# bpp/bpp

Hardware: AMD Instinct MI355X
Metric: MCMC iterations/sec (A00) + site-lnL updates/sec, 10k loci, 1/2/4/8 GPU (higher is better)
Workload: dtype f64; 1 GPU; C2: A00, 10000 loci x 1000 sites, 4 taxa, JC69, 1 rate cat; 10000 loci on rank 0, 5.2 patterns/locus; parallelism=1 GPU, moves=program

## Files before the change

### bpp_amd/csrc/sweep2.hpp

```cpp
#pragma once

namespace smp2 {

using smp::Tree; using smp::Species; using smp::ByteArr; using smp::MAXPOP; using smp::MAXN;
using smp::rndu; using smp::reflect; using smp::msc_term; using smp::nth_bit; using smp::Op; using smp::make_op;

template <int NT> struct Cfg
{
  static constexpr int G     = NT <= 4 ? 8 : NT <= 8 ? 16 : 32;
  static constexpr int LPW   = 64/G;
  static constexpr int NN    = 2*NT;
  static constexpr int W     = NN/4;
  static constexpr int NBUF  = 2*(NT - 1);
  static constexpr int NPM   = 2*(2*NT - 2);
#ifndef SMP2_WAVES
#define SMP2_WAVES 8
#endif
  static constexpr int WAVES = NT <= 4 ? SMP2_WAVES : 4;
  static constexpr int BS    = 64*WAVES;
  static constexpr int PARK  = 28 + 4*W;
  static_assert(G == NN, "lane i of a group is node i");
};

struct Loc
// ... 32 lines not shown
  const Sched * sched; uint32_t sched_on;
  uint32_t xshards;
};

constexpr int XV = 15;
constexpr uint32_t XS_MIN = 8, XS_MAX = 64, XLINE = 16;
constexpr size_t XBUF_WORDS = (size_t)2*XS_MAX*XLINE;
constexpr int XSLEEP_FIRST = 16;
struct XLayout { uint32_t set_words, shard, word; };
__host__ __device__ inline XLayout xlayout(uint32_t S, uint32_t b, uint32_t lane, uint32_t load)
{
  XLayout L;
  L.set_words = S*XLINE;
  L.shard = (b & (S - 1u))*XLINE;
  L.word = ((lane >> 4) + 4u*load)*XLINE + (lane & 15u);
  return L;
}
template <int NL> __device__ __forceinline__ unsigned long long xpoll_sum(const unsigned long long * p, uint32_t step)
{
  unsigned long long v[NL];
#pragma unroll
  for (int j = 0; j < NL; ++j) v[j] = __hip_atomic_load(p + (size_t)j*step, __ATOMIC_RELAXED, __HIP_MEMORY_SCOPE_AGENT);
  unsigned long long s = v[0];
#pragma unroll
  for (int j = 1; j < NL; ++j) s += v[j];
  return s;
}

template <int NT> struct Slot
{
  double time[Cfg<NT>::NN];
  double ab[Cfg<NT>::NPM][2];
  double contrib[Cfg<NT>::G], contrib_new[Cfg<NT>::G];
  double rate, rw, f[4];
};
template <int NT> struct WaveLDS
{
  double clv[Cfg<NT>::NBUF][64][4];
  double term[64];
  uint2  pat[64];
  Slot<NT> slot[Cfg<NT>::LPW];
};
struct PopFit { double k, T, a, b, c; };
struct Redraw { double tn, l2t, T, a, b, c; };
struct WgBase
{
  double tau[3*MAXPOP];
  double xtot[32];
  Species sp;
  struct { unsigned long long grng; uint32_t accm, rd_mask, acc_step, run_ok; double lnacc_step, lnacc_theta; double tn[16], l2t[16], lnacc[16]; } dec;
  PopFit pf[16];
  Redraw rd[16];
  struct { int32_t q, mix; double tq_old, tq_lo, tq_hi, tq_new, minf, maxf, lminf, lmaxf, mix_c, mix_lnc; } stepp;
};
template <int NT> struct WgLDS : WgBase
{
  double lograt[(2*NT)*(2*NT)];
  unsigned long long accfx[32];
  uint32_t anc[16];
  uint32_t abort_, bad_, xbad_, coarse_;
  unsigned long long xprev[2][64];
  long long prof[24];
  long long wsweep[16];
  uint32_t roles[8];
  uint32_t xcoarse_, late_;
  uint32_t simd[8];
  uint32_t handoff[8][SCHED_SEGS];
  unsigned long long b1abs; long long hwait[8], b1last;
};

template <int G> __device__ __forceinline__ uint32_t gballot(bool p, uint32_t gbase)
{
  return (uint32_t)(__ballot(p) >> gbase) & (G >= 32 ? 0xffffffffu : ((1u << (G & 31)) - 1u));
}
__device__ __forceinline__ void wsync()
{
  __builtin_amdgcn_fence(__ATOMIC_ACQ_REL, "wavefront");
  __builtin_amdgcn_wave_barrier();
}

template <int NT> struct GTree
{
  ByteArr<Cfg<NT>::W> left, right, parent, pop;
  uint32_t cf, pf;
  int32_t root, tips;
  __device__ __forceinline__ int cidx(int i) const { return i + (((cf >> i) & 1u) ? tips - 1 : 0); }
  __device__ __forceinline__ int pidx(int i) const { return i + (((pf >> i) & 1u) ? 2*tips - 2 : 0); }
};

__device__ __forceinline__ uint32_t splat(int v) { return (uint32_t)(v & 0xff)*0x01010101u; }
__device__ __forceinline__ uint32_t byte_eq(uint32_t w, uint32_t s)
{
  const uint32_t x = w ^ s;
  const uint32_t z = ~(((x & 0x7f7f7f7fu) + 0x7f7f7f7fu) | x | 0x7f7f7f7fu);
  return (z - (z >> 7)) | z;
}
template <int NT> __device__ __forceinline__ void swap_ids(GTree<NT> & t, double * time, int a, int b)
{
  constexpr int W = Cfg<NT>::W;
  const uint32_t sa = splat(a), sb = splat(b), x = sa ^ sb;
#pragma unroll
  for (int k = 0; k < W; ++k)
  {
    t.left.w[k]   ^= x & (byte_eq(t.left.w[k], sa)   | byte_eq(t.left.w[k], sb));
    t.right.w[k]  ^= x & (byte_eq(t.right.w[k], sa)  | byte_eq(t.right.w[k], sb));
    t.parent.w[k] ^= x & (byte_eq(t.parent.w[k], sa) | byte_eq(t.parent.w[k], sb));
  }
  const int la = t.left[a], ra = t.right[a], pa = t.parent[a], qa = t.pop[a];
  const int lb = t.left[b], rb = t.right[b], pb = t.parent[b], qb = t.pop[b];
  t.left.set(a, lb); t.right.set(a, rb); t.parent.set(a, pb); t.pop.set(a, qb);
  t.left.set(b, la); t.right.set(b, ra); t.parent.set(b, pa); t.pop.set(b, qa);
  const double ta = time[a], tb = time[b];
  time[a] = tb; time[b] = ta;
  t.root = t.root == a ? b : t.root == b ? a : t.root;
}
template <int NT> __device__ __forceinline__ uint32_t path_mask(const GTree<NT> & t, int v)
{
  uint32_t m = 0;
#pragma unroll
  for (int d = 0; d < NT; ++d) { if (v >= 0) { m |= 1u << v; v = t.parent[v]; } }
  return m;
}

// ... 390 lines not shown
  const uint32_t lane = threadIdx.x & 63u, pl16 = lane & 15u, role = lane >> 4;
  const int npop = wg.sp.npop, pm = (int)pl16;
  const double qnan = prog_qnan();
  const bool run_ok = wg.dec.run_ok != 0u;
  const PopFit f = wg.pf[pl16];
  const bool have = lane < 32u && pm < npop && ((theta_mask >> pm) & 1u) && run_ok;
  const double Ts = f.T*mix_c;
  double fa = qnan, fb = qnan, tn = qnan, l2t = 0;
  if (have) theta_conditional<TK>(wg, f.k, role == 0u ? Ts : Ts/mix_c, &fa, &fb);
  const double fao = __shfl(fa, 16 + pm, 64), fbo = __shfl(fb, 16 + pm, 64);
  const uint32_t rd_mask = (uint32_t)__ballot(lane < 16u && have && fa == fa && fao == fao) & 0xffffu;
  double xl;
  const double s_fa = __shfl(fa, pm, 64), s_fb = __shfl(fb, pm, 64);
  const double g = draw_gammas<TK>(z, lane, 0xfedcba9876543210ull, npop, rd_mask, fa, role == 1u ? s_fb : role == 2u ? s_fa : fbo, xl);
  const double lb = __shfl(xl, 16 + pm, 64), la = __shfl(xl, 32 + pm, 64), lbo = __shfl(xl, 48 + pm, 64), lao = log(fao);
  const double c1 = fa*lb - lgamma_with_log(fa, la), co = fao*lbo - lgamma_with_log(fao, lao);
  if (lane < 16u && ((rd_mask >> pl16) & 1u)) tn = 1.0/(g/fb);
  const double x = redraw_ratio<TK>(wg, lane, f.k, tn, fa, fb, c1, Ts, fao, fbo, co, f.T, l2t);
  double lnacc_theta = 0;
  for (int p = 0; p < npop; ++p)
    if ((theta_mask >> p) & 1u)
    {
      const double xp = __shfl(x, p, 64);
      lnacc_theta += run_ok && ((rd_mask >> p) & 1u) ? xp : qnan;
    }
  if (lane < 16u) { Redraw & r = wg.rd[lane]; r.tn = tn; r.l2t = l2t; r.T = Ts; r.a = fa; r.b = fb; r.c = c1; }
  if (lane == 0) { wg.dec.rd_mask = rd_mask; wg.dec.lnacc_theta = lnacc_theta; }
  __builtin_amdgcn_fence(__ATOMIC_ACQ_REL, "wavefront");
  __builtin_amdgcn_wave_barrier();
  return z;
}

template <int NT, bool BPP, bool PROG = false, bool HO = false>
__global__ void __launch_bounds__(Cfg<NT>::BS) iter_kernel(const Args A)
{
  static_assert(!HO || PROG, "sets change waves in the program-moves kernel only");
  using C = Cfg<NT>;
  constexpr int G = C::G, LPW = C::LPW, NN = C::NN, W = C::W, NBUF = C::NBUF, NPM = C::NPM, WAVES = C::WAVES;
  extern __shared__ __attribute__((aligned(16))) unsigned char smem[];
  WgLDS<NT> & wg = *reinterpret_cast<WgLDS<NT> *>(smem);
  WaveLDS<NT> * wl_all = reinterpret_cast<WaveLDS<NT> *>(smem + ((sizeof(WgLDS<NT>) + 15) & ~(size_t)15));
  const uint32_t tid = threadIdx.x, wv = tid >> 6, lane = tid & 63u, b = blockIdx.x;
  const int li = (int)(lane & (uint32_t)(G - 1)); const uint32_t gbase = lane - (uint32_t)li, slot = lane/(uint32_t)G;
  const uint32_t lw = PROG ? wv - 1u : wv;
  WaveLDS<NT> * wl = wl_all + (PROG ? (wv && !(HO && wv > A.lwaves) ? wv - 1u : 0u) : wv);
  Slot<NT> * S = &wl->slot[slot];
  const uint32_t gw = lw < A.lwaves ? b*A.lwaves + lw : 0xffffffffu;
  {
    const uint32_t * src = reinterpret_cast<const uint32_t *>(A.sp);
    uint32_t * dst = reinterpret_cast<uint32_t *>(&wg.sp);
    for (uint32_t i = tid; i < sizeof(Species)/4; i += C::BS) dst[i] = src[i];
    if (tid < 24u) wg.prof[tid] = 0;
    if (tid < 16u) wg.wsweep[tid] = 0;
    if constexpr (HO)
    {
      if (tid < 8u) { wg.hwait[tid] = 0; wg.roles[tid] = 0xff0u; }
      if (tid < 8u*SCHED_SEGS) (&wg.handoff[0][0])[tid] = 0u;
      if (tid == 0) { wg.b1last = 0; wg.b1abs = 0ull; }
      if (lane == 0) wg.simd[wv & 7u] = (uint32_t)__builtin_amdgcn_s_getreg((1 << 11) | (4 << 6) | 4);
    }
  }
  __syncthreads();
  const Species & SP = wg.sp;
  const int npop = SP.npop, nsp = SP.S;

  for (uint32_t i = tid; i < (uint32_t)(3*MAXPOP); i += C::BS) wg.tau[i] = A.taus[i];
  for (uint32_t i = tid; i < (uint32_t)((2*NT)*(2*NT)); i += C::BS) wg.lograt[i] = A.lograt[(i/(2*NT))*MAXN + i % (2*NT)];
  if (tid < 16u) wg.anc[tid] = tid < (uint32_t)MAXPOP ? (uint32_t)SP.anc[tid] : 0u;
  if (tid == 0) { wg.abort_ = __hip_atomic_load(A.err, __ATOMIC_RELAXED, __HIP_MEMORY_SCOPE_AGENT) != 0 ? 2u : 0u; wg.late_ = 0; wg.bad_ = 0; wg.xbad_ = 0; wg.coarse_ = 0; wg.xcoarse_ = 0; }
  if (tid < 32u) wg.accfx[tid] = 0ull;
  if (tid < 2u*64u) (&wg.xprev[0][0])[tid] = 0ull;
  PopLane pl;
  {
    pl.parent = li < npop ? (int)SP.parent[li < MAXPOP ? li : 0] : -1;
    pl.anc = li < npop ? (uint32_t)SP.anc[li < MAXPOP ? li : 0] : 0u;
    uint32_t below = 0;
    for (int q2 = 0; q2 < npop; ++q2) if (q2 != li && (((uint32_t)SP.anc[q2] >> li) & 1u)) below |= 1u << q2;
    pl.below = li < npop ? below : 0u;
  }
  __syncthreads();
  if (wg.abort_ == 2u)
  {
    if (b == 0 && tid == 0) (void)atomicAdd(A.err + 1, (int)A.niter);
    return;
  }
  auto load_pop = [&]()
  {
    const int i = li < MAXPOP ? li : 0;
    pl.tau = wg.tau[i]; pl.theta = wg.tau[MAXPOP + i]; pl.l2t = wg.tau[2*MAXPOP + i];
    pl.ptau = pl.parent >= 0 ? wg.tau[pl.parent] : -1.0;
  };
  load_pop();
  Stream<BPP> grng{*A.grng};

  const bool prof_on = (A.dbg & 16u) && b == 0 && tid == 0;
  long long pf_t = prof_on ? clock64() : 0;
#define SMP2_TICK(i_) do { if (prof_on) { const long long t1_ = clock64(); wg.prof[i_] += t1_ - pf_t; pf_t = t1_; } } while (0)
  long long pf_s = 0;
#define SMP2_SUB0() do { if (prof_on) pf_s = clock64(); } while (0)
#define SMP2_SUB(i_) do { if (prof_on) wg.prof[i_] += clock64() - pf_s; } while (0)

  constexpr double FX = 1099511627776.0;
  constexpr double FXC = 1024.0;
  auto fx_add = [&](int v, double x, bool coarse)
  {
    if (fabs(x) < 256.0)
// ... 168 lines not shown
      uint32_t pj_tau = 0, pj_tau_acc = 0, pj_mix = 0, pj_mix_acc = 0;
      const bool declog = (A.dbg & 256u) && b == 0;
      int q = -1; bool mix = false;
      double tq_old = 0, tq_new = 0, mix_c = 1, mix_lnc = 0, lnprior = 0;
      auto make_step = [&](int stepq)
      {
        mix = stepq == npop; q = mix ? -1 : stepq;
        const double wprop = g.window();
        double tq_lo = 0, tq_hi = 0, minf = 1, maxf = 1, lminf = 0, lmaxf = 0;
        tq_old = 0; tq_new = 0; mix_c = 1; mix_lnc = 0; lnprior = 0;
        if (!mix)
        {
          const int pq = SP.parent[q], cl = SP.left[q], cr = SP.right[q];
          tq_old = wg.tau[q]; tq_lo = fmax(wg.tau[cl], wg.tau[cr]); tq_hi = pq >= 0 ? wg.tau[pq] : 999.0;
          tq_new = reflect(tq_old + SP.ft_tau*wprop, tq_lo, tq_hi);
          minf = (tq_new - tq_lo)/(tq_old - tq_lo); maxf = (tq_new - tq_hi)/(tq_old - tq_hi);
          const double lg = log(lane == 0 ? minf : lane == 1u ? maxf : tq_new/tq_old);
          lminf = __shfl(lg, 0, 64); lmaxf = __shfl(lg, 1, 64);
          if (pq < 0 && SP.tau_alpha > 0) lnprior = (SP.tau_alpha - 1 - (nsp - 1) + 1)*__shfl(lg, 2, 64) - SP.tau_beta*(tq_new - tq_old);
        }
        else { mix_lnc = SP.ft_mix*wprop; mix_c = exp(mix_lnc); }
        if (lane == 0)
        {
          wg.stepp.q = q; wg.stepp.mix = mix ? 1 : 0; wg.stepp.tq_old = tq_old; wg.stepp.tq_lo = tq_lo; wg.stepp.tq_hi = tq_hi; wg.stepp.tq_new = tq_new;
          wg.stepp.minf = minf; wg.stepp.maxf = maxf; wg.stepp.lminf = lminf; wg.stepp.lmaxf = lmaxf; wg.stepp.mix_c = mix_c; wg.stepp.mix_lnc = mix_lnc;
        }
      };
      uint32_t slidem = 0; double tslide = 0;
      auto theta_choices = [&]()
      {
        slidem = 0; tslide = 0;
        for (int p = 0; p < npop; ++p)
          if ((tm >> p) & 1u)
          {
            if (!(g.u() < SP.theta_slide_prob)) continue;
            slidem |= 1u << p;
            const double tn = reflect(wg.tau[MAXPOP + p] + SP.ft_theta*g.window(), 0.0, 999.0);
            if (p == (int)lane) tslide = tn;
          }
      };
      bool aborted = false;
      if (A.do_allloci && A.niter) { make_step(nsp); theta_choices(); }
      __syncthreads();
      for (uint32_t it = 0; it < A.niter && A.do_allloci && !aborted; ++it)
      {
        for (int stepq = nsp; stepq <= npop && !aborted; ++stepq)
        {
          const bool first = stepq == nsp;
          const int base = first ? nth : 0;
          if (mix) { SMP2_SUB0(); g.r = prog_mix_redraw((uint32_t)g.r, tm, mix_c); SMP2_SUB(15); }
          SMP2_TICK(0);
          __syncthreads();
          SMP2_TICK(1);
          if constexpr (HO) if (wg.abort_) { if (b == 0 && lane == 0) (void)atomicAdd(A.err + 1, (int)A.niter); aborted = true; __syncthreads(); __syncthreads(); break; }
          double dummy = 0;
          exchange_begin(base + (mix ? 2 : 5));
          SMP2_TICK(2);
          const bool okx = exchange_end(0, dummy);
          SMP2_TICK(3);
          if (!okx) { aborted = true; __syncthreads(); __syncthreads(); break; }
          if ((A.dbg & 64u) && A.world == 1)
          {
            xdummy = true; xrow = 16;
            exchange_begin(base + (mix ? 2 : 5));
            const bool okd = exchange_end(0, dummy);
            xdummy = false; xrow = 8;
            if (!okd) { aborted = true; __syncthreads(); __syncthreads(); break; }
            if (prof_on) pf_t = clock64();
          }
          bool accept = false; double lnacc = 0; uint32_t rd_mask = 0;
          if (first)
          {
            g.r = prog_theta_decide((uint32_t)g.r, tm, slidem, tslide, 1, q, base);
            const uint32_t accm = wg.dec.accm;
            cnt_prop += (uint32_t)__popc(tm); cnt_acc += (uint32_t)__popc(accm);
            cnt_gprop += (uint32_t)__popc(tm & ~slidem); cnt_gacc += (uint32_t)__popc(accm & tm & ~slidem);
            if (declog && lane < (uint32_t)npop && ((tm >> lane) & 1u))
            {
              const uint32_t k = ndec + (uint32_t)__popc(tm & ((1u << lane) - 1u));
              if (k < 1000u) { double * r = A.declog + 4*k; r[0] = (((slidem >> lane) & 1u) ? 100 : 200) + (int)lane; r[1] = wg.dec.lnacc[lane]; r[2] = -1.0; r[3] = (accm >> lane) & 1u ? 1 : 0; }
            }
            ndec += (uint32_t)__popc(tm);
            SMP2_TICK(4);
          }
          if (!mix)
          {
            g.r = prog_tau_decide((uint32_t)g.r, tm, q, base, lnprior, first);
            accept = wg.dec.acc_step != 0u; rd_mask = wg.dec.rd_mask; lnacc = wg.dec.lnacc_step;
          }
          else
          {
            lnacc = (wg.xtot[0] + wg.xtot[1]*(FX/FXC)) + (double)(nsp - 1)*mix_lnc;
            if (SP.tau_alpha > 0)
            {
              const double troot = wg.tau[npop - 1];
              lnacc += (SP.tau_alpha - 1)*mix_lnc - SP.tau_beta*(troot*mix_c - troot) - (double)(nsp - 2)*mix_lnc;
            }
            lnacc += wg.dec.lnacc_theta; rd_mask = wg.dec.rd_mask;
            accept = g.accept(lnacc);
            if (lane == 0) wg.dec.acc_step = accept ? 1u : 0u;
          }
          if (accept && wg.xcoarse_ && b == 0 && lane == 0) (void)atomicAdd(A.err + 2, 1);
          ++cnt_prop; cnt_acc += accept ? 1u : 0u;
          if (mix) { ++pj_mix; pj_mix_acc += accept ? 1u : 0u; } else { ++pj_tau; pj_tau_acc += accept ? 1u : 0u; }
          if (declog && lane == 0 && ndec < 1000u) { double * r = A.declog + 4*ndec; r[0] = mix ? 300 : 200 + q; r[1] = lnacc; r[2] = -1.0; r[3] = accept ? 1 : 0; }
          ++ndec;
          if (accept)
          {
            if (!mix) { if (lane == 0) wg.tau[q] = tq_new; }
            else if (lane < (uint32_t)npop) wg.tau[lane] *= mix_c;
            if (lane < 16u)
            {
              const Redraw r = wg.rd[lane];
              if ((rd_mask >> lane) & 1u) { wg.tau[MAXPOP + lane] = r.tn; wg.tau[2*MAXPOP + lane] = r.l2t; }
              const bool moved = mix ? lane < (uint32_t)npop && ((tm >> lane) & 1u)
                                     : ((tm >> lane) & 1u) && ((int)lane == q || (int)lane == SP.left[q] || (int)lane == SP.right[q]);
              if (moved) { PopFit & f = wg.pf[lane]; f.T = r.T; f.a = r.a; f.b = r.b; f.c = r.c; }
            }
          }
          wsync();
          if (mix) SMP2_TICK(6); else SMP2_TICK(5);
          SMP2_TICK(7);
          __syncthreads();
          if (stepq < npop) make_step(stepq + 1);
          else if (it + 1 < A.niter) { make_step(nsp); theta_choices(); }
          __syncthreads();
        }
      }
      if (!aborted)
      {
        if (lane == 0) wg.late_ = __hip_atomic_load(A.err, __ATOMIC_ACQUIRE, __HIP_MEMORY_SCOPE_AGENT) != 0 ? 1u : 0u;
        __syncthreads();
        if (wg.late_) { aborted = true; if (b == 0 && lane == 0) (void)atomicAdd(A.err + 1, (int)A.niter); }
      }
      if (b == 0)
      {
        if (lane == 0 && !aborted)
        {
          *A.grng = g.r;
          A.counters[0] += cnt_prop; A.counters[1] += cnt_acc; A.counters[2] += cnt_gprop; A.counters[3] += cnt_gacc;
          A.pj[4] += pj_tau; A.pj[5] += pj_tau_acc; A.pj[6] += pj_mix; A.pj[7] += pj_mix_acc;
          A.pj[8] += (cnt_prop - pj_tau - pj_mix) - cnt_gprop; A.pj[9] += (cnt_acc - pj_tau_acc - pj_mix_acc) - cnt_gacc;
        }
        if (!aborted && lane < (uint32_t)(3*MAXPOP)) A.taus[lane] = wg.tau[lane];
        if (prof_on) for (int i = 0; i < 24; ++i) A.prof[(i < 16 ? 0 : (int)A.nwg) + i] = (double)wg.prof[i];
        if (prof_on) for (int i = 0; i < 16; ++i) A.prof[(int)A.nwg + 24 + i] = (double)wg.wsweep[i];
        if (HO && prof_on) { for (int i = 0; i < 8; ++i) { A.prof[(int)A.nwg + 40 + i] = (double)wg.hwait[i]; A.prof[(int)A.nwg + 49 + i] = (double)wg.roles[i]; } A.prof[(int)A.nwg + 48] = (double)wg.b1last; }
      }
      return;
    }
  }

  const uint32_t t0 = gw < A.nwaves ? A.wave_off[gw] : 0u, nt = gw < A.nwaves ? A.wave_off[gw + 1] - t0 : 0u;
  bool act = slot < nt;
  uint32_t task = t0 + (act ? slot : 0u);
  GTree<NT> T;
  Stream<BPP> rng{0};
  double lnl_cur = 0, logpr_cur = 0;
  uint32_t np = 0, pb = 0, nprop_done = 0, nacc = 0, w_nupd = 0, w_nbr = 0, a_nupd = 0, a_nbr = 0, a_neval = 0;
  int gl_i = 0;
  for (int k = 0; k < W; ++k) { T.left.w[k] = T.right.w[k] = T.parent.w[k] = T.pop.w[k] = 0xffffffffu; }
  T.cf = T.pf = 0; T.root = 0; T.tips = 2;
  if (act && nt)
  {
    const Loc & L = A.loc[task];
    const uint32_t flag_now = __hip_atomic_load(A.mix_flag, __ATOMIC_RELAXED, __HIP_MEMORY_SCOPE_AGENT);
    const bool restore_mix = A.epoch != 0u && flag_now == A.epoch;
    const Tree * trp = A.trees + task;
    if (restore_mix) trp = A.snap + task;
    const Tree & tr = *trp;
    const Tree & cur = A.trees[task];
    np = L.np;
    double * g_pmat = L.pmat;
    if (li == 0) { S->rate = L.rate; S->rw = L.rw; S->f[0] = L.f0; S->f[1] = L.f1; S->f[2] = L.f2; S->f[3] = L.f3; }
    gl_i = L.gl[li & 15];
    for (int k = 0; k < W; ++k)
    {
      T.left.w[k] = reinterpret_cast<const uint32_t *>(tr.left)[k]; T.right.w[k] = reinterpret_cast<const uint32_t *>(tr.right)[k];
      T.parent.w[k] = reinterpret_cast<const uint32_t *>(tr.parent)[k]; T.pop.w[k] = reinterpret_cast<const uint32_t *>(tr.pop)[k];
// ... 2 lines not shown
    const int n = 2*T.tips - 1;
    T.cf = gballot<G>(li >= T.tips && li < n && tr.clv[li] != li, gbase);
    T.pf = gballot<G>(li < n && tr.pmat[li] != li, gbase);
    S->time[li] = li < n ? tr.time[li] : 0.0;
    for (uint32_t i = (uint32_t)li; i < (uint32_t)(4*(2*T.tips - 2)); i += G) (&S->ab[0][0])[i] = g_pmat[i];
  }
  {
    uint32_t acc = 0;
#pragma unroll
    for (int s2 = 0; s2 < LPW; ++s2)
    {
      const uint32_t n2 = (uint32_t)__builtin_amdgcn_readlane((int)np, s2*G);
      if ((uint32_t)s2 == slot) pb = acc;
      acc += n2;
    }
  }
  if (act)
  {
    const Loc & L = A.loc[task];
    const double * g_clv = L.clv;
    for (uint32_t q = (uint32_t)li; q < np; q += G) wl->pat[pb + q] = A.pat[L.pat_off + q];
    const uint32_t nbuf = 2u*(uint32_t)(T.tips - 1);
    for (uint32_t i = (uint32_t)li; i < nbuf*np; i += G)
    {
      const uint32_t c = i/np, q = i - c*np;
      const double2 * src = reinterpret_cast<const double2 *>(g_clv + ((size_t)c*np + q)*4);
      const double2 u = src[0], w = src[1];
      double * d = wl->clv[c][pb + q];
      d[0] = u.x; d[1] = u.y; d[2] = w.x; d[3] = w.y;
    }
  }
  int tips = T.tips, n = 2*tips - 1;
  bool inner_i = li >= tips && li < n;

  uint32_t mync = 0; double t2h_cur = 0, t2h_new = 0;
  uint32_t mynodes = 0, mync_new = 0; int mynin_new = 0;
  Op opw[NT - 1]; int nops = 0;
  for (int k = 0; k < NT - 1; ++k) opw[k] = 0;

  auto density_counts = [&]()
  {
    const int pop_i = T.pop[li];
    int below = 0;
#pragma unroll
    for (int q = 0; q < G - 1; ++q)
    {
      const uint32_t m = gballot<G>(inner_i && pop_i == q, gbase);
      if (li == q) mynodes = m;
      below += ((pl.below >> q) & 1u) ? __popc(m) : 0;
    }
    mync_new = (uint32_t)__popc(mynodes);
    mynin_new = gl_i - below;
  };
  auto density_term = [&](const double * tk)
  {
    uint32_t nodes = mynodes;
    const int ncoal = (int)mync_new, nin = mynin_new;
    int steps = ncoal + (pl.ptau >= 0 ? 1 : 0);
    if (nin == steps) --steps;
    double T2h = 0, prev = pl.tau;
    int nn = nin;
#pragma unroll
    for (int k = 0; k < NT; ++k)
      if (k < steps)
      {
        double tkk = pl.ptau;
        if (k < ncoal)
        {
          int best = -1; double tb = 0;
#pragma unroll
          for (int j = 0; j < NT - 1; ++j)
            if (((nodes >> (tips + j)) & 1u) && (best < 0 || tk[j] < tb)) { best = tips + j; tb = tk[j]; }
          tkk = tb; nodes &= ~(1u << best);
        }
        T2h += nn*(nn - 1)*(tkk - prev);
        prev = tkk; --nn;
      }
    double c = 0;
    if (ncoal) c += ncoal*pl.l2t;
    if (T2h) c -= T2h/(pl.theta*1.0);
    S->contrib_new[li] = c; t2h_new = T2h;
  };
  auto evaluate = [&](const Prop & pr, bool with_lnl, double & lp_new) -> double
  {
    double tk[NT - 1];
#pragma unroll
    for (int j = 0; j < NT - 1; ++j) tk[j] = S->time[(tips + j) & (NN - 1)];
    const double myage = S->time[li];
    density_counts();
    if ((pr.chain >> li) & 1u) density_term(tk);
    T.pf ^= pr.brm; T.cf ^= pr.ndm;
    if ((pr.brm >> li) & 1u)
    {
      const int par = T.parent[li];
      const double len = (S->time[par & (NN - 1)] - myage)*1.0;
      double a_, b_;
      jc69_ab(len, S->rate, a_, b_);
      const int pi = T.pidx(li);
      S->ab[pi][0] = a_; S->ab[pi][1] = b_;
    }
    nops = __popc(pr.ndm);
    {
      int rank = 0;
#pragma unroll
      for (int j = 0; j < NT - 1; ++j)
        rank += (((pr.ndm >> (tips + j)) & 1u) && (tk[j] < myage || (tk[j] == myage && tips + j < li))) ? 1 : 0;
      const bool mine = (pr.ndm >> li) & 1u;
#pragma unroll
      for (int k = 0; k < NT - 1; ++k)
        if (k < nops)
        {
          const int x = __ffs(gballot<G>(mine && rank == k, gbase)) - 1;
          const int l = T.left[x], r = T.right[x];
          opw[k] = make_op(T.cidx(x), T.cidx(l), T.pidx(l), T.cidx(r), T.pidx(r));
        }
    }
    wsync();
    double lnl = 0;
    if (with_lnl)
    {
      for (uint32_t base = 0; base < np; base += G)
      {
        const uint32_t q = base + (uint32_t)li; const bool pact = q < np;
        const uint32_t ps = pb + (pact ? q : 0u);
        const uint2 pi = wl->pat[ps];
        double last[4] = {0, 0, 0, 0}; uint32_t last_c = 0xffffffffu;
#pragma unroll
        for (int k = 0; k < NT - 1; ++k)
          if (k < nops)
          {
            const Op o = opw[k];
            const uint32_t opar = (uint32_t)o & 255u, lc = (uint32_t)(o >> 8) & 255u, lp = (uint32_t)(o >> 16) & 255u,
                           rc = (uint32_t)(o >> 24) & 255u, rp = (uint32_t)(o >> 32) & 255u;
            double lv[4], rv[4], x[4], y[4];
            if (lc < (uint32_t)tips) expand_code((pi.y >> (4*lc)) & 15u, lv);
            else if (lc == last_c) { lv[0] = last[0]; lv[1] = last[1]; lv[2] = last[2]; lv[3] = last[3]; }
            else { const double * c = wl->clv[lc - tips][ps]; lv[0] = c[0]; lv[1] = c[1]; lv[2] = c[2]; lv[3] = c[3]; }
            if (rc < (uint32_t)tips) expand_code((pi.y >> (4*rc)) & 15u, rv);
            else if (rc == last_c) { rv[0] = last[0]; rv[1] = last[1]; rv[2] = last[2]; rv[3] = last[3]; }
            else { const double * c = wl->clv[rc - tips][ps]; rv[0] = c[0]; rv[1] = c[1]; rv[2] = c[2]; rv[3] = c[3]; }
            matvec4_ab(S->ab[lp][0], S->ab[lp][1], lv, x);
            matvec4_ab(S->ab[rp][0], S->ab[rp][1], rv, y);
            last[0] = x[0]*y[0]; last[1] = x[1]*y[1]; last[2] = x[2]*y[2]; last[3] = x[3]*y[3]; last_c = opar;
            if (pact) { double * out = wl->clv[opar - tips][ps]; out[0] = last[0]; out[1] = last[1]; out[2] = last[2]; out[3] = last[3]; }
          }
        const double tr_ = dot4_pair(S->f[0], S->f[1], S->f[2], S->f[3], last);
        if (pact) wl->term[ps] = log(0 + tr_*S->rw)*pi.x;
      }
      wsync();
      for (uint32_t base = 0; base < np; base += 8)
      {
        double v[8];
#pragma unroll
        for (int j = 0; j < 8; ++j) v[j] = base + (uint32_t)j < np ? wl->term[pb + base + (uint32_t)j] : 0.0;
#pragma unroll
        for (int j = 0; j < 8; ++j) lnl += v[j];
      }
      lnl = A.bfbeta == 1.0 ? lnl : A.bfbeta == 0.0 ? 0.0 : A.bfbeta*lnl;
    }
    else wsync();
    double lp = 0;
    {
      double v[G];
#pragma unroll
      for (int p = 0; p < G; ++p) v[p] = p < npop ? (((pr.chain >> p) & 1u) ? S->contrib_new[p] : S->contrib[p]) : 0.0;
#pragma unroll
      for (int p = 0; p < G; ++p) lp += v[p];
    }
    lp_new = lp;
    return lnl;
  };
  auto commit_density = [&](uint32_t chain)
  {
    if ((chain >> li) & 1u) { S->contrib[li] = S->contrib_new[li]; t2h_cur = t2h_new; }
    mync = mync_new;
  };

  const uint32_t allpop = (1u << npop) - 1u;
  if (act)
  {
    wsync();
    double tk[NT - 1];
#pragma unroll
    for (int j = 0; j < NT - 1; ++j) tk[j] = S->time[(tips + j) & (NN - 1)];
    density_counts();
    if (li < npop) density_term(tk);
    commit_density(allpop);
    wsync();
    if (A.refresh_logpr)
    {
      double lp = 0;
      for (int p = 0; p < npop; ++p) lp += S->contrib[p];
      logpr_cur = lp;
    }
  }

  const double qnan = __longlong_as_double(0x7ff8000000000000ll);
  uint32_t cnt_prop = 0, cnt_acc = 0;
  uint32_t cnt_gprop = 0, cnt_gacc = 0;
  uint32_t pj_tau = 0, pj_tau_acc = 0, pj_mix = 0, pj_mix_acc = 0, pj_gage = 0, pj_gage_acc = 0;
  uint32_t step = 0;

  if constexpr (HO)
  {
    uint32_t role = 0xffu; bool handover = false;
    if (A.sched_on && lw < A.lwaves && A.lwaves <= 7u)
    {
      const uint32_t L = A.lwaves;
      uint32_t nalone = 0; bool valid = true;
      for (uint32_t x = 0; x < L; ++x)
      {
        uint32_t cnt = 0;
        for (uint32_t y = 0; y < L; ++y) cnt += (y != x && wg.simd[y + 1u] == wg.simd[x + 1u]) ? 1u : 0u;
        valid = valid && cnt <= 1u;
        nalone += cnt == 0u ? 1u : 0u;
      }
      uint32_t ia = 0, ip = 0;
      for (uint32_t x = 0; x < L; ++x)
      {
        int partner = -1;
        for (uint32_t y = 0; y < L; ++y) if (y != x && wg.simd[y + 1u] == wg.simd[x + 1u]) partner = (int)y;
        if (partner < 0) { if (x == lw) role = ia; ++ia; }
        else if ((uint32_t)partner > x)
        {
          if (x == lw) role = nalone + 2u*ip;
          if ((uint32_t)partner == lw) role = nalone + 2u*ip + 1u;
          ++ip;
        }
      }
      handover = valid && ip == (uint32_t)A.sched->npairs && nalone + 2u*ip == (uint32_t)A.sched->nroles && role < 8u;
    }
    if (lane == 0) wg.roles[wv & 7u] = wg.simd[wv & 7u] | (role << 4) | (handover ? 0x1000u : 0u);
    wsync();
  }
  auto park = [&]()
  {
    if constexpr (HO) {
    const uint32_t myset = (uint32_t)(wl - wl_all);
    uint32_t * r = reinterpret_cast<uint32_t *>(wl_all + A.lwaves) + (size_t)myset*(C::PARK*64) + lane;
// ... 55 lines not shown
      act = false;
      if (lane == 0) wg.roles[wv & 7u] &= ~0x1000u;
    }
    wsync();
    }
  };
  auto segment_begin = [&](uint32_t seg, uint32_t it, uint32_t nprop, bool prof) -> uint32_t
  {
    if constexpr (HO)
    {
      const uint32_t role = (wg.roles[wv & 7u] >> 4) & 7u;
      const uint32_t nseg = A.sched->nseg, src = A.sched->src[role][seg & 3u], nrun = A.sched->n[role][seg & 3u];
      if (seg && src != role) hand_over(role, src, seg, it, prof);
      return (wg.roles[wv & 7u] & 0x1000u) && seg + 1u < nseg && step + nrun < nprop ? step + nrun : nprop;
    }
    return nprop;
  };
  const bool declog = (A.dbg & 256u) && b == 0;
  uint32_t ndec = 0;
  const bool wgprof = (A.dbg & 32u) && tid == 0;
  long long wg_sweep = 0;
  bool aborted = false;

  if constexpr (PROG) __syncthreads();
  for (uint32_t it = 0; it < A.niter && !aborted; ++it)
  {
    const uint32_t nprop = HO && lw >= A.lwaves ? 0u : A.nsteps_gage + A.nsteps_gspr;
    const long long wg_t0 = wgprof ? clock64() : 0;
    const bool wvprof = (A.dbg & 16u) && b == 0 && lane == 0;
    const long long wv_t0 = wvprof ? clock64() : 0;
    step = 0;
    uint32_t seg = 0;
    do
    {
    uint32_t seg_end = nprop;
    if constexpr (HO) { if (wg.roles[wv & 7u] & 0x1000u) seg_end = segment_begin(seg, it, nprop, wvprof); ++seg; }
    for (; step < seg_end; ++step)
    {
      const GTree<NT> U = T;
      double tsave = 0, lnl = 0, lp_new = 0;
      Prop pr{0, 0, 0, 0.0};
      bool ok = false;
      if (act)
      {
        tsave = S->time[li];
        ok = step < A.nsteps_gage
          ? propose_gage<NT, BPP>(T, rng, S->time, (int)step, pl, wg.anc, wg.tau, SP.ft_gage, li, gbase, pr)
          : propose_gspr<NT, BPP>(T, rng, S->time, (int)(step - A.nsteps_gage), pl, gl_i, wg.anc, wg.tau, wg.lograt, SP.ft_gspr, li, gbase, pr);
      }
      SMP2_TICK(0);
      if (ok)
      {
        wsync();
        lnl = evaluate(pr, true, lp_new);
        SMP2_TICK(1);
      }
      if (ok)
      {
        w_nupd += (uint32_t)nops; w_nbr += (uint32_t)__popc(pr.brm);
        const double lnacc = (lp_new - logpr_cur) + (lnl - lnl_cur) + pr.hast;
        ++nprop_done;
        const bool gage_step = step < A.nsteps_gage;
        pj_gage += gage_step ? 1u : 0u;
        if (rng.accept(lnacc)) { lnl_cur = lnl; logpr_cur = lp_new; ++nacc; pj_gage_acc += gage_step ? 1u : 0u; commit_density(pr.chain); }
        else { T = U; S->time[li] = tsave; }
        wsync();
        SMP2_TICK(2);
      }
      else if (act) { T = U; S->time[li] = tsave; wsync(); }
    }
    } while (HO && step < nprop);
    (void)seg;
    if (wgprof) wg_sweep += clock64() - wg_t0;
    if (wvprof)
    {
      const long long t1 = clock64();
      wg.wsweep[wv] += t1 - wv_t0;
      if constexpr (HO) (void)__hip_atomic_fetch_max(&wg.b1abs, (unsigned long long)t1, __ATOMIC_RELAXED, __HIP_MEMORY_SCOPE_WORKGROUP);
    }
    if (!A.do_allloci) continue;

    constexpr bool program = PROG;
    bool mix = false; int q = -1;
    double wprop = 0, uacc = -1.0;
    double tq_old = 0, tq_lo = 0, tq_hi = 0, minf = 1, maxf = 1, lminf = 0, lmaxf = 0, tq_new = 0, mix_c = 1, mix_lnc = 0;
    double lnacc_theta = 0;
    double rd_tn = qnan, rd_l2t = 0, rd_T = 0, rd_a = qnan, rd_b = qnan, rd_c = qnan;
    uint32_t rd_mask = 0;
    uint32_t cf0 = 0, pf0 = 0;
    double tsave = 0, lnl_new = 0, lp_new = 0, lnprior = 0, dl_tot = 0, lnacc = 0;
    bool evaluated = false, accept = false;
    auto step_begin = [&](int stepq)
    {
      rd_mask = 0; lnprior = 0; accept = false; lnacc_theta = 0;
      if constexpr (PROG)
      {
        (void)stepq;
        mix = wg.stepp.mix != 0; q = wg.stepp.q;
        tq_old = wg.stepp.tq_old; tq_lo = wg.stepp.tq_lo; tq_hi = wg.stepp.tq_hi; tq_new = wg.stepp.tq_new;
        minf = wg.stepp.minf; maxf = wg.stepp.maxf; lminf = wg.stepp.lminf; lmaxf = wg.stepp.lmaxf; mix_c = wg.stepp.mix_c; mix_lnc = wg.stepp.mix_lnc;
      }
      else
      {
        mix = stepq == npop;
        q = mix ? -1 : stepq;
        wprop = mix && !BPP ? grng.u() - 0.5 : grng.window(); uacc = BPP ? -1.0 : grng.u();
        tq_old = 0; tq_lo = 0; tq_hi = 0; minf = 1; maxf = 1; lminf = 0; lmaxf = 0; tq_new = 0; mix_c = 1; mix_lnc = 0;
        if (!mix)
        {
          const int pq = SP.parent[q], cl = SP.left[q], cr = SP.right[q];
          tq_old = wg.tau[q]; tq_lo = fmax(wg.tau[cl], wg.tau[cr]); tq_hi = pq >= 0 ? wg.tau[pq] : 999.0;
          tq_new = reflect(tq_old + SP.ft_tau*wprop, tq_lo, tq_hi);
          minf = (tq_new - tq_lo)/(tq_old - tq_lo); maxf = (tq_new - tq_hi)/(tq_old - tq_hi);
          lminf = log(minf); lmaxf = log(maxf);
        }
        else { mix_lnc = SP.ft_mix*wprop; mix_c = exp(mix_lnc); }
      }
      if (!mix)
      {
        if (li == q) pl.tau = tq_new;
        if (pl.parent == q) pl.ptau = tq_new;
      }
      else
      {
        pl.tau *= mix_c;
        if (pl.parent >= 0) pl.ptau *= mix_c;
      }
    };
    auto step_locus = [&](int base)
    {
      cf0 = T.cf; pf0 = T.pf;
      tsave = act ? S->time[li] : 0.0;
      lnl_new = lnl_cur; lp_new = logpr_cur;
      evaluated = false;
      if (act)
      {
        Prop pr{allpop, 0, 0, 0.0};
        double hast = 0, hast2 = 0;
        if (!mix)
        {
          const int cl = SP.left[q], cr = SP.right[q];
          const int pk = T.pop[li];
          const double tk_ = tsave;
          const bool moved = inner_i && (pk == q || pk == cl || pk == cr) && !(tk_ < tq_lo || tk_ > tq_hi);
          const bool up = moved && tk_ >= tq_old;
          if (moved) S->time[li] = up ? tq_hi + maxf*(tk_ - tq_hi) : tq_lo + minf*(tk_ - tq_lo);
          const uint32_t mm = gballot<G>(moved, gbase);
          const int above = __popc(gballot<G>(up, gbase)), below = __popc(mm) - above;
          const int par = T.parent[li];
          pr.brm = gballot<G>(li < n && par >= 0 && (((mm >> li) & 1u) || ((mm >> (par & 31)) & 1u)), gbase);
          uint32_t m = mm;
          const int l = T.left[li], r = T.right[li];
#pragma unroll
          for (int d = 0; d < NT - 2; ++d) m |= gballot<G>(inner_i && (((m >> (l & 31)) & 1u) || ((m >> (r & 31)) & 1u)), gbase);
          pr.ndm = m;
          hast = below*lminf; hast2 = above*lmaxf;
        }
        else
        {
          if (inner_i) S->time[li] = tsave*mix_c;
          pr.ndm = gballot<G>(inner_i, gbase);
          pr.brm = gballot<G>(li < n && (int)T.parent[li] >= 0, gbase);
          hast = (double)(tips - 1)*mix_lnc;
        }
        wsync();
        evaluated = pr.ndm != 0;
        const double lnl = evaluate(pr, evaluated, lp_new);
        if (evaluated) { lnl_new = lnl; a_nupd += (uint32_t)nops; a_nbr += (uint32_t)__popc(pr.brm); ++a_neval; }
        const double dpr = program ? 0.0 : lp_new - logpr_cur;
        const double h = mix ? dpr + hast : (dpr + hast) + hast2;
        const double dl = evaluated ? (lnl_new - lnl_cur) + h : h;
        if (li == 0) fx_add(base, dl, true);
        if (program && !mix && li < npop && ((A.theta_mask >> li) & 1u))
        {
          const int slot = li == q ? 2 : li == SP.left[q] ? 3 : li == SP.right[q] ? 4 : -1;
          if (slot >= 0) fx_add(base + slot, t2h_new, false);
        }
      }
    };
    auto step_decide = [&](int base)
    {
      dl_tot = wg.xtot[base] + wg.xtot[base + 1]*(FX/FXC);
      lnacc = dl_tot;
      if (!mix) lnacc += lnprior;
      else
      {
        lnacc += (double)(nsp - 1)*mix_lnc;
        if (SP.tau_alpha > 0)
        {
          const double troot = wg.tau[npop - 1];
          lnacc += (SP.tau_alpha - 1)*mix_lnc - SP.tau_beta*(troot*mix_c - troot) - (double)(nsp - 2)*mix_lnc;
        }
      }
      accept = BPP ? grng.accept(lnacc) : (lnacc >= 0 || uacc < exp(lnacc));
    };
    auto step_apply = [&](bool refresh)
    {
      if constexpr (!PROG)
      {
        if (accept && wg.xcoarse_ && b == 0 && tid == 0) (void)atomicAdd(A.err + 2, 1);
        ++cnt_prop; cnt_acc += accept ? 1u : 0u;
        if (mix) { ++pj_mix; pj_mix_acc += accept ? 1u : 0u; } else { ++pj_tau; pj_tau_acc += accept ? 1u : 0u; }
        if (declog && tid == 0 && ndec < 1000u) { double * r = A.declog + 4*ndec; r[0] = mix ? 300 : 200 + q; r[1] = lnacc; r[2] = uacc; r[3] = accept ? 1 : 0; }
        ++ndec;
        __syncthreads();
        if (accept)
        {
          if (!mix) { if (tid == 0) wg.tau[q] = tq_new; }
          else if (tid < (uint32_t)npop) wg.tau[tid] *= mix_c;
        }
      }
      if (accept) { if (act) { lnl_cur = lnl_new; logpr_cur = lp_new; commit_density(allpop); } }
      else if (act) { T.cf = cf0; T.pf = pf0; S->time[li] = tsave; }
      if constexpr (!PROG) __syncthreads();
      load_pop();
      wsync();
      if (PROG && (refresh || accept) && act)
      {
        if (li < npop) S->contrib[li] = msc_term((int)mync, t2h_cur, pl.theta, pl.l2t);
        wsync();
        double lp = 0;
        for (int p = 0; p < npop; ++p) lp += S->contrib[p];
        logpr_cur = lp;
        wsync();
      }
    };
    if constexpr (PROG)
    {
      const bool on = li < npop && ((A.theta_mask >> li) & 1u);
      const int kidx = __popc(A.theta_mask & ((1u << li) - 1u)), nth = 2*__popc(A.theta_mask);
      for (int stepq = nsp; stepq <= npop && !aborted; ++stepq)
      {
        const bool first = stepq == nsp;
        step_begin(stepq);
        if (first && act && on) { fx_add(2*kidx, (double)mync, false); fx_add(2*kidx + 1, t2h_cur, false); }
        step_locus(first ? nth : 0);
        __syncthreads();
        if constexpr (HO) if (first && wvprof && lw == 0u) wg.b1last += (long long)wg.b1abs - wv_t0;
        __syncthreads();
        const bool ab = wg.abort_ != 0u;
        accept = wg.dec.acc_step != 0u;
        if (!ab) step_apply(first);
        __syncthreads();
        if (ab) { aborted = true; break; }
      }
    }
    else
    {
    if (SP.theta_alpha > 0 && A.theta_mask)
    {
      const bool on = li < npop && ((A.theta_mask >> li) & 1u);
      const double told = pl.theta, l2t_old = pl.l2t;
      double tnew = told, uacc = -1.0, my_lnacc = 0;
      bool accept = false, gibbs_me = false;
      {
        double win = 0;
        for (int p = 0; p < npop; ++p)
          if ((A.theta_mask >> p) & 1u)
          {
            const double w_ = grng.window(), a_ = BPP ? -1.0 : grng.u();
            if (p == li) { win = w_; uacc = a_; }
          }
        tnew = reflect(told + SP.ft_theta*win, 0.0, 999.0);
        const double l2t_new = log(2.0/(1.0*tnew));
        if (act && on) fx_add(li, msc_term((int)mync, t2h_cur, tnew, l2t_new) - msc_term((int)mync, t2h_cur, told, l2t_old), false);
        SMP2_TICK(3);
        double th_tot = 0;
        if (!exchange(npop, li, th_tot)) { aborted = true; break; }
        SMP2_TICK(6);
        if (BPP)
        {
          if (on) { wl->term[li] = tnew; wl->term[16 + li] = told; }
          wsync();
          for (int p = 0; p < npop; ++p)
            if ((A.theta_mask >> p) & 1u)
            {
              const double tn = wl->term[p], to = wl->term[16 + p];
              const double lnacc = wg.xtot[p] + ((SP.theta_alpha - 1)*log(tn/to) - SP.theta_beta*(tn - to));
              const bool acc = tn > 0 && grng.accept(lnacc);
              if (p == li) { accept = acc; my_lnacc = lnacc; }
            }
          wsync();
        }
        else if (on)
        {
          my_lnacc = th_tot + ((SP.theta_alpha - 1)*log(tnew/told) - SP.theta_beta*(tnew - told));
          accept = tnew > 0 && (my_lnacc >= 0 || uacc < exp(my_lnacc));
        }
      }
      const double l2t_new = log(2.0/(1.0*tnew));
      if (accept) { pl.theta = tnew; pl.l2t = l2t_new; }
      if (declog && tid < (uint32_t)G && on)
      {
        const uint32_t k = ndec + (uint32_t)__popc(A.theta_mask & ((1u << li) - 1u));
        if (k < 2048u) { double * r = A.declog + 4*k; r[0] = (gibbs_me ? 200 : 100) + li; r[1] = my_lnacc; r[2] = uacc; r[3] = accept ? 1 : 0; }
      }
      ndec += (uint32_t)__popc(A.theta_mask);
      {
        const uint32_t onm = gballot<G>(on, gbase), accm = gballot<G>(accept, gbase), gm = gballot<G>(on && gibbs_me, gbase);
        cnt_prop += (uint32_t)__popc(onm); cnt_acc += (uint32_t)__popc(accm);
        cnt_gprop += (uint32_t)__popc(gm); cnt_gacc += (uint32_t)__popc(gm & accm);
      }
      __syncthreads();
      if (tid < (uint32_t)G && accept) { wg.tau[MAXPOP + li] = tnew; wg.tau[2*MAXPOP + li] = l2t_new; }
      __syncthreads();
      if (act)
      {
        if (li < npop) S->contrib[li] = msc_term((int)mync, t2h_cur, pl.theta, pl.l2t);
        wsync();
        double lp = 0;
        for (int p = 0; p < npop; ++p) lp += S->contrib[p];
        logpr_cur = lp;
        wsync();
      }
    }
    SMP2_TICK(3);

    for (int stepq = nsp; stepq <= npop && !aborted; ++stepq)
    {
      step_begin(stepq);
      step_locus(0);
      if (mix) SMP2_TICK(5); else SMP2_TICK(4);
      if (!mix && SP.parent[q] < 0 && SP.tau_alpha > 0)
        lnprior = (SP.tau_alpha - 1 - (nsp - 1) + 1)*log(tq_new/tq_old) - SP.tau_beta*(tq_new - tq_old);
      if (!exchange(2, 0, dl_tot)) { aborted = true; break; }
      if (A.dbg & 64u) { SMP2_TICK(7); double dummy; if (!exchange(2, 0, dummy)) { aborted = true; break; } SMP2_TICK(6); }
      SMP2_TICK(7);
      SMP2_SUB0();
      step_decide(0);
      SMP2_SUB(14);
      step_apply(false);
      if (mix) SMP2_TICK(5); else SMP2_TICK(4);
    }
    }
  }
#undef SMP2_TICK
#undef SMP2_SUB0
#undef SMP2_SUB
  if (aborted || wg.abort_) return;
  if constexpr (!PROG) { if (tid == 0) wg.late_ = __hip_atomic_load(A.err, __ATOMIC_ACQUIRE, __HIP_MEMORY_SCOPE_AGENT) != 0 ? 1u : 0u; }
  __syncthreads();
  if (wg.late_)
  {
    if constexpr (!PROG) { if (b == 0 && tid == 0) (void)atomicAdd(A.err + 1, (int)A.niter); }
    return;
  }

  if (act)
  {
    Tree & tr = A.trees[task];
    double * g_clv = A.loc[task].clv, * g_pmat = A.loc[task].pmat;
    {
      uint32_t wl_ = 0, wr_ = 0, wp_ = 0, wq_ = 0;
#pragma unroll
      for (int k = 0; k < W; ++k) if (li == k) { wl_ = T.left.w[k]; wr_ = T.right.w[k]; wp_ = T.parent.w[k]; wq_ = T.pop.w[k]; }
      if (li < W)
      {
        reinterpret_cast<uint32_t *>(tr.left)[li] = wl_; reinterpret_cast<uint32_t *>(tr.right)[li] = wr_;
        reinterpret_cast<uint32_t *>(tr.parent)[li] = wp_; reinterpret_cast<uint32_t *>(tr.pop)[li] = wq_;
      }
    }
    if (li < n) { tr.time[li] = S->time[li]; tr.clv[li] = (int8_t)T.cidx(li); tr.pmat[li] = (int8_t)T.pidx(li); }
    if (li == 0)
    {
      tr.lnl = lnl_cur; tr.logpr = logpr_cur; tr.rng = rng.r; tr.root = T.root;
      tr.proposals += nprop_done; tr.accepted += nacc; tr.sw_nupd += w_nupd; tr.sw_nbr += w_nbr;
      tr.al_nupd += a_nupd; tr.al_nbr += a_nbr; tr.al_neval += a_neval;
      (void)atomicAdd(A.pj + 0, (unsigned long long)pj_gage); (void)atomicAdd(A.pj + 1, (unsigned long long)pj_gage_acc);
      (void)atomicAdd(A.pj + 2, (unsigned long long)(nprop_done - pj_gage)); (void)atomicAdd(A.pj + 3, (unsigned long long)(nacc - pj_gage_acc));
    }
    if (li < npop) { A.pop_nc[(size_t)li*A.ntasks + task] = (int8_t)mync; A.pop_t2h[(size_t)li*A.ntasks + task] = t2h_cur; }
    for (uint32_t i = (uint32_t)li; i < (uint32_t)(4*(2*tips - 2)); i += G) g_pmat[i] = (&S->ab[0][0])[i];
    const uint32_t nbuf = 2u*(uint32_t)(tips - 1);
    for (uint32_t i = (uint32_t)li; i < nbuf*np; i += G)
// ... 27 lines not shown
```

Baseline: 8803 iterations/s.

## Skip per-step prior density sums in program-moves path and add iteration handshake

In the program-moves kernel, the per-locus evaluate no longer computes per-population prior contributions or sums lp_new. On accept it only copies t2h, and density counts are recomputed only on the first step of each sweep. The prior refresh now runs only when requested rather than on every accept. A workgroup-scope iteration counter with a sleep-spin wait, timeout and abort is added so locus waves do not start an iteration before the decision wave has prepared its step parameters. The abort check is also made unconditional. Together this removes redundant density arithmetic and wave syncs per step, at the cost of a new spin-wait handshake and the risk of stale density state.

Result: faster. 9094 iterations/s, median of 6 (+3.3%).

```diff
diff --git a/bpp_amd/csrc/sweep2.hpp b/bpp_amd/csrc/sweep2.hpp
--- a/bpp_amd/csrc/sweep2.hpp
+++ b/bpp_amd/csrc/sweep2.hpp
@@ -108,6 +108,7 @@
   PopFit pf[16];
   Redraw rd[16];
   struct { int32_t q, mix; double tq_old, tq_lo, tq_hi, tq_new, minf, maxf, lminf, lmaxf, mix_c, mix_lnc; } stepp;
+  uint32_t stepp_iter, pad_;
 };
 template <int NT> struct WgLDS : WgBase
 {
@@ -122,9 +123,11 @@
   uint32_t xcoarse_, late_;
   uint32_t simd[8];
   uint32_t handoff[8][SCHED_SEGS];
+  unsigned long long twait[8];
   unsigned long long b1abs; long long hwait[8], b1last;
 };
 
+template <bool B> struct BoolC { static constexpr bool value = B; };
 template <int G> __device__ __forceinline__ uint32_t gballot(bool p, uint32_t gbase)
 {
   return (uint32_t)(__ballot(p) >> gbase) & (G >= 32 ? 0xffffffffu : ((1u << (G & 31)) - 1u));
@@ -621,6 +624,7 @@
     for (uint32_t i = tid; i < sizeof(Species)/4; i += C::BS) dst[i] = src[i];
     if (tid < 24u) wg.prof[tid] = 0;
     if (tid < 16u) wg.wsweep[tid] = 0;
+    if constexpr (PROG) { if (tid == 0) wg.stepp_iter = 0u; }
     if constexpr (HO)
     {
       if (tid < 8u) { wg.hwait[tid] = 0; wg.roles[tid] = 0xff0u; }
@@ -895,7 +899,7 @@
           SMP2_TICK(0);
           __syncthreads();
           SMP2_TICK(1);
-          if constexpr (HO) if (wg.abort_) { if (b == 0 && lane == 0) (void)atomicAdd(A.err + 1, (int)A.niter); aborted = true; __syncthreads(); __syncthreads(); break; }
+          if (wg.abort_) { if (b == 0 && lane == 0) (void)atomicAdd(A.err + 1, (int)A.niter); aborted = true; __syncthreads(); __syncthreads(); break; }
           double dummy = 0;
           exchange_begin(base + (mix ? 2 : 5));
           SMP2_TICK(2);
@@ -966,8 +970,12 @@
           SMP2_TICK(7);
           __syncthreads();
           if (stepq < npop) make_step(stepq + 1);
-          else if (it + 1 < A.niter) { make_step(nsp); theta_choices(); }
           __syncthreads();
+          if (stepq == npop && it + 1 < A.niter)
+          {
+            make_step(nsp); theta_choices();
+            if (lane == 0) __hip_atomic_store(&wg.stepp_iter, it + 1u, __ATOMIC_RELEASE, __HIP_MEMORY_SCOPE_WORKGROUP);
+          }
         }
       }
       if (!aborted)
@@ -1076,7 +1084,7 @@
     mync_new = (uint32_t)__popc(mynodes);
     mynin_new = gl_i - below;
   };
-  auto density_term = [&](const double * tk)
+  auto density_term = [&](const double * tk, auto stat)
   {
     uint32_t nodes = mynodes;
     const int ncoal = (int)mync_new, nin = mynin_new;
@@ -1100,19 +1108,24 @@
         T2h += nn*(nn - 1)*(tkk - prev);
         prev = tkk; --nn;
       }
-    double c = 0;
-    if (ncoal) c += ncoal*pl.l2t;
-    if (T2h) c -= T2h/(pl.theta*1.0);
-    S->contrib_new[li] = c; t2h_new = T2h;
+    if constexpr (!decltype(stat)::value)
+    {
+      double c = 0;
+      if (ncoal) c += ncoal*pl.l2t;
+      if (T2h) c -= T2h/(pl.theta*1.0);
+      S->contrib_new[li] = c;
+    }
+    t2h_new = T2h;
   };
-  auto evaluate = [&](const Prop & pr, bool with_lnl, double & lp_new) -> double
-  {
+  auto evaluate = [&](const Prop & pr, bool with_lnl, double & lp_new, auto stat) -> double
+  {
+    constexpr bool STAT = decltype(stat)::value;
     double tk[NT - 1];
 #pragma unroll
     for (int j = 0; j < NT - 1; ++j) tk[j] = S->time[(tips + j) & (NN - 1)];
     const double myage = S->time[li];
-    density_counts();
-    if ((pr.chain >> li) & 1u) density_term(tk);
+    if constexpr (!STAT) density_counts();
+    if ((pr.chain >> li) & 1u) density_term(tk, stat);
     T.pf ^= pr.brm; T.cf ^= pr.ndm;
     if ((pr.brm >> li) & 1u)
     {
@@ -1183,15 +1196,16 @@
       lnl = A.bfbeta == 1.0 ? lnl : A.bfbeta == 0.0 ? 0.0 : A.bfbeta*lnl;
     }
     else wsync();
-    double lp = 0;
-    {
+    if constexpr (!STAT)
+    {
+      double lp = 0;
       double v[G];
 #pragma unroll
       for (int p = 0; p < G; ++p) v[p] = p < npop ? (((pr.chain >> p) & 1u) ? S->contrib_new[p] : S->contrib[p]) : 0.0;
 #pragma unroll
       for (int p = 0; p < G; ++p) lp += v[p];
-    }
-    lp_new = lp;
+      lp_new = lp;
+    }
     return lnl;
   };
   auto commit_density = [&](uint32_t chain)
@@ -1208,7 +1222,7 @@
 #pragma unroll
     for (int j = 0; j < NT - 1; ++j) tk[j] = S->time[(tips + j) & (NN - 1)];
     density_counts();
-    if (li < npop) density_term(tk);
+    if (li < npop) density_term(tk, BoolC<false>{});
     commit_density(allpop);
     wsync();
     if (A.refresh_logpr)
@@ -1370,7 +1384,7 @@
       if (ok)
       {
         wsync();
-        lnl = evaluate(pr, true, lp_new);
+        lnl = evaluate(pr, true, lp_new, BoolC<false>{});
         SMP2_TICK(1);
       }
       if (ok)
@@ -1397,6 +1411,28 @@
       if constexpr (HO) (void)__hip_atomic_fetch_max(&wg.b1abs, (unsigned long long)t1, __ATOMIC_RELAXED, __HIP_MEMORY_SCOPE_WORKGROUP);
     }
     if (!A.do_allloci) continue;
+    if constexpr (PROG)
+    {
+      if (it && __hip_atomic_load(&wg.stepp_iter, __ATOMIC_ACQUIRE, __HIP_MEMORY_SCOPE_WORKGROUP) != it)
+      {
+        if (lane == 0) wg.twait[wv & 7u] = wall_clock64();
+        wsync();
+        for (uint32_t rounds = 1;; ++rounds)
+        {
+          __builtin_amdgcn_s_sleep(1);
+          if (__hip_atomic_load(&wg.stepp_iter, __ATOMIC_ACQUIRE, __HIP_MEMORY_SCOPE_WORKGROUP) == it) break;
+          bool give_up = __hip_atomic_load(&wg.abort_, __ATOMIC_RELAXED, __HIP_MEMORY_SCOPE_WORKGROUP) != 0u;
+          if (!give_up && (rounds & 63u) == 0)
+            give_up = wall_clock64() - wg.twait[wv & 7u] > 50000000ull || __hip_atomic_load(A.err, __ATOMIC_RELAXED, __HIP_MEMORY_SCOPE_AGENT) != 0;
+          if (give_up)
+          {
+            if (lane == 0) { __hip_atomic_store(&wg.abort_, 1u, __ATOMIC_RELAXED, __HIP_MEMORY_SCOPE_WORKGROUP); (void)__hip_atomic_exchange(A.err, 1, __ATOMIC_RELEASE, __HIP_MEMORY_SCOPE_AGENT); }
+            act = false;
+            break;
+          }
+        }
+      }
+    }
 
     constexpr bool program = PROG;
     bool mix = false; int q = -1;
@@ -1445,7 +1481,7 @@
         if (pl.parent >= 0) pl.ptau *= mix_c;
       }
     };
-    auto step_locus = [&](int base)
+    auto step_locus = [&](int base, bool counts)
     {
       cf0 = T.cf; pf0 = T.pf;
       tsave = act ? S->time[li] : 0.0;
@@ -1483,7 +1519,9 @@
         }
         wsync();
         evaluated = pr.ndm != 0;
-        const double lnl = evaluate(pr, evaluated, lp_new);
+        double lnl;
+        if constexpr (PROG) { if (counts) density_counts(); lnl = evaluate(pr, evaluated, lp_new, BoolC<true>{}); }
+        else lnl = evaluate(pr, evaluated, lp_new, BoolC<false>{});
         if (evaluated) { lnl_new = lnl; a_nupd += (uint32_t)nops; a_nbr += (uint32_t)__popc(pr.brm); ++a_neval; }
         const double dpr = program ? 0.0 : lp_new - logpr_cur;
         const double h = mix ? dpr + hast : (dpr + hast) + hast2;
@@ -1528,12 +1566,16 @@
           else if (tid < (uint32_t)npop) wg.tau[tid] *= mix_c;
         }
       }
-      if (accept) { if (act) { lnl_cur = lnl_new; logpr_cur = lp_new; commit_density(allpop); } }
+      if (accept)
+      {
+        if constexpr (PROG) { if (act) { lnl_cur = lnl_new; if (li < npop) t2h_cur = t2h_new; } }
+        else if (act) { lnl_cur = lnl_new; logpr_cur = lp_new; commit_density(allpop); }
+      }
       else if (act) { T.cf = cf0; T.pf = pf0; S->time[li] = tsave; }
       if constexpr (!PROG) __syncthreads();
       load_pop();
       wsync();
-      if (PROG && (refresh || accept) && act)
+      if (PROG && refresh && act)
       {
         if (li < npop) S->contrib[li] = msc_term((int)mync, t2h_cur, pl.theta, pl.l2t);
         wsync();
@@ -1552,13 +1594,13 @@
         const bool first = stepq == nsp;
         step_begin(stepq);
         if (first && act && on) { fx_add(2*kidx, (double)mync, false); fx_add(2*kidx + 1, t2h_cur, false); }
-        step_locus(first ? nth : 0);
+        step_locus(first ? nth : 0, first);
         __syncthreads();
         if constexpr (HO) if (first && wvprof && lw == 0u) wg.b1last += (long long)wg.b1abs - wv_t0;
         __syncthreads();
         const bool ab = wg.abort_ != 0u;
         accept = wg.dec.acc_step != 0u;
-        if (!ab) step_apply(first);
+        if (!ab) step_apply(stepq == npop);
         __syncthreads();
         if (ab) { aborted = true; break; }
       }
@@ -1637,7 +1679,7 @@
     for (int stepq = nsp; stepq <= npop && !aborted; ++stepq)
     {
       step_begin(stepq);
-      step_locus(0);
+      step_locus(0, false);
       if (mix) SMP2_TICK(5); else SMP2_TICK(4);
       if (!mix && SP.parent[q] < 0 && SP.tau_alpha > 0)
         lnprior = (SP.tau_alpha - 1 - (nsp - 1) + 1)*log(tq_new/tq_old) - SP.tau_beta*(tq_new - tq_old);
```
